# facebookresearch/mbrl-lib

Measured on AMD Instinct MI355X. Metric: candidate-steps/sec (pop×particles×horizon / plan) per CEM iter; plans/sec, higher is better.
Workload: dtype f32

## Files before the change

### __graft_entry__.py

```python
import os
import subprocess
import sys

ROOT = os.path.dirname(os.path.abspath(__file__))
PKG = os.path.join(ROOT, "mbrl-lib_amd")
CSRC = os.path.join(PKG, "csrc")
LIB = os.path.join(PKG, "hipets", "libhipets.so")
BUILDINFO = os.path.join(PKG, "hipets", "libhipets.buildinfo.json")
OBJDIR = os.path.join(PKG, "build")
HIPCC = os.environ.get("HIPCC", "/opt/rocm/bin/hipcc")
HOST_UNITS = ["train.hip", "plan.hip", "rollout.hip", "model.hip", "comm.hip", "engine.hip"]
UNITS = ["rollout_r3.hip", "rollout_r4_gen.hip", "rollout_r4_gens.hip", "rollout_r3_gen.hip", "rollout_r3_gens.hip", "rollout_r2.hip", "rollout_r2_gen.hip",
         "rollout_r2_gens.hip", "rollout_r1_gen.hip", "rollout_r1_gens.hip", "rollout_r1.hip", "rollout_r4.hip", "rollout_r2_fast.hip", "rollout_r3_fast.hip",
         "rollout_r1_fast.hip", "planet.hip"] + HOST_UNITS + ["rollout_r4_fast.hip"]
FLAGS = ["--offload-arch=gfx950", "-O3", "-std=c++17", "-ffp-contract=off", "-fPIC", "-Wno-pass-failed"]


def _sources():
    return sorted(os.path.join(CSRC, f) for f in os.listdir(CSRC)) + [os.path.join(ROOT, "include", "hipets.h")]


def source_digest(extra_flags=()):
    import hashlib

# ... 209 lines not shown
            if "argument unused during compilation" not in line:
                print(line, file=sys.stderr)
        if proc.returncode != 0:
            raise subprocess.CalledProcessError(proc.returncode, cmd)
        stem = os.path.basename(o)[:-2]
        for f in os.listdir(objdir):
            if (f.startswith(stem + "-") or f.startswith(stem + ".")) and f != stem + ".o":
                path = os.path.join(objdir, f)
                if f.endswith("gfx950.s"):
                    resources.update(parse_kernel_resources(path))
                    n, found = scan_isa_hazards(path)
                    isa["asm_mfmas"] += n
                    isa["hazards"] += found
                    isa["units_scanned"].append(u)
                os.remove(path)

    with ThreadPoolExecutor(max_workers=min(len(UNITS), os.cpu_count() or 1)) as ex:
        list(ex.map(lambda uo: compile_unit(*uo), zip(UNITS, objs)))
    link_extra = [f for f in extra_flags if f.startswith("-fsanitize") or f in ("-fno-gpu-sanitize", "-shared-libsan")]
    cmd = [HIPCC, "--offload-arch=gfx950", "-shared", "-fPIC"] + link_extra + objs + ["-o", out]
    print("[build]", " ".join(cmd), flush=True)
    subprocess.run(cmd, check=True)
    with open(os.path.splitext(out)[0] + ".buildinfo.json", "w") as f:
        json.dump({"source_digest": digest, "flags": FLAGS + list(extra_flags), "units": UNITS, "kernels": resources, "isa": isa}, f)
    for h in isa["hazards"][:20]:
        print("[build] ISA HAZARD:", h, file=sys.stderr)
    if isa["hazards"] and not os.environ.get("HIPETS_ALLOW_ISA_HAZARDS") and "-O1" not in extra_flags:
        raise RuntimeError(f"{len(isa['hazards'])} ISA hazard finding(s) in {out}: see {os.path.splitext(out)[0]}.buildinfo.json")
    return digest


DEBUG_LIB = os.path.join(PKG, "hipets", "libhipets_debug.so")
ASAN_LIB = os.path.join(PKG, "hipets", "libhipets_asan.so")
DEBUG_OBJDIR = os.path.join(PKG, "build_debug")
DEBUG_FLAGS = ["-O1", "-gline-tables-only", "-DHIPETS_DEBUG_BOUNDS=1"]
ASAN_FLAGS = ["-fsanitize=address", "-fno-gpu-sanitize", "-shared-libsan", "-Wno-option-ignored"]


def asan_runtime() -> str:
    out = subprocess.run([HIPCC, "--print-file-name=libclang_rt.asan-x86_64.so"], capture_output=True, text=True).stdout.strip()
    if not os.path.isabs(out) or not os.path.exists(out):
        import glob

        found = sorted(glob.glob("/opt/rocm/lib/llvm/lib/clang/*/lib/linux/libclang_rt.asan-x86_64.so"))
        out = found[-1] if found else out
    return out


def build_debug(force: bool = False) -> str:
    import json

    digest = source_digest(DEBUG_FLAGS)
    rebuilt = built_digest(DEBUG_LIB) != digest or force
    build_library(out=DEBUG_LIB, extra_flags=DEBUG_FLAGS, objdir=DEBUG_OBJDIR, force=force)
    asan_digest = source_digest(DEBUG_FLAGS + ASAN_FLAGS)
    if rebuilt or built_digest(ASAN_LIB) != asan_digest:
        from concurrent.futures import ThreadPoolExecutor

        def compile_asan(u):
            obj = os.path.join(DEBUG_OBJDIR, u.replace(".hip", "_asan.o"))
            cmd = [HIPCC] + FLAGS + DEBUG_FLAGS + ASAN_FLAGS + ["-c", os.path.join(CSRC, u), "-o", obj]
            print("[build]", " ".join(cmd), flush=True)
            subprocess.run(cmd, check=True)
            return obj

        with ThreadPoolExecutor(max_workers=min(len(HOST_UNITS), os.cpu_count() or 1)) as ex:
            objs = list(ex.map(compile_asan, HOST_UNITS))
        others = [os.path.join(DEBUG_OBJDIR, u.replace(".hip", ".o")) for u in UNITS if u not in HOST_UNITS]
        cmd = [HIPCC, "--offload-arch=gfx950", "-shared", "-fPIC", "-fsanitize=address", "-fno-gpu-sanitize", "-shared-libsan"] + objs + others + ["-o", ASAN_LIB]
        print("[build]", " ".join(cmd), flush=True)
        subprocess.run(cmd, check=True)
        with open(os.path.splitext(ASAN_LIB)[0] + ".buildinfo.json", "w") as f:
            json.dump({"source_digest": asan_digest, "flags": FLAGS + DEBUG_FLAGS + ASAN_FLAGS, "units": UNITS}, f)
    return DEBUG_LIB


def build(force: bool = False, debug: bool = True) -> None:
    build_library(force=force)
    if debug and os.environ.get("HIPETS_BUILD_DEBUG", "1") != "0":
        build_debug(force)
    build_c_client(force)
    build_fake_rccl(force)
    build_residency_harness(force)
    for p in (PKG, ROOT):
        if p not in sys.path:
            sys.path.insert(0, p)
    import hipets
    from hipets import _lib

    _lib.load()
    from oracle import pets_oracle


C_CLIENT_SRC = os.path.join(ROOT, "tests", "c_abi", "plan_from_c.c")
C_CLIENT = os.path.join(ROOT, "tests", "c_abi", "plan_from_c")


def build_c_client(force: bool = False) -> None:
    if not force and os.path.exists(C_CLIENT) and os.path.getmtime(C_CLIENT) >= max(os.path.getmtime(C_CLIENT_SRC), os.path.getmtime(LIB)):
        return
    cmd = ["gcc", "-std=c99", "-Wall", "-Wextra", "-Werror", "-O1", C_CLIENT_SRC, "-I" + os.path.join(ROOT, "include"),
           "-I/opt/rocm/include", "-D__HIP_PLATFORM_AMD__", "-L" + os.path.dirname(LIB), "-lhipets", "-L/opt/rocm/lib",
           "-lamdhip64", "-lm", "-Wl,-rpath,$ORIGIN/../../mbrl-lib_amd/hipets", "-Wl,-rpath,/opt/rocm/lib", "-o", C_CLIENT]
    print("[build]", " ".join(cmd), flush=True)
    subprocess.run(cmd, check=True)


FAKE_RCCL_SRC = os.path.join(ROOT, "tests", "fake_rccl", "fake_rccl.cpp")
FAKE_RCCL = os.path.join(ROOT, "tests", "fake_rccl", "libfake_rccl.so")


def build_fake_rccl(force: bool = False) -> str:
    if force or not os.path.exists(FAKE_RCCL) or os.path.getmtime(FAKE_RCCL) < os.path.getmtime(FAKE_RCCL_SRC):
        cmd = ["g++", "-std=c++17", "-shared", "-fPIC", "-O1", "-Wall", "-Wextra", FAKE_RCCL_SRC, "-I/opt/rocm/include",
               "-D__HIP_PLATFORM_AMD__", "-L/opt/rocm/lib", "-lamdhip64", "-lrt", "-lpthread", "-Wl,-rpath,/opt/rocm/lib", "-o", FAKE_RCCL]
        print("[build]", " ".join(cmd), flush=True)
        subprocess.run(cmd, check=True)
    return FAKE_RCCL


RESIDENCY_HARNESS_SRC = os.path.join(ROOT, "tests", "residency", "rule_harness.cpp")
RESIDENCY_HARNESS = os.path.join(ROOT, "tests", "residency", "rule_harness")


def build_residency_harness(force: bool = False) -> str:
    srcs = [RESIDENCY_HARNESS_SRC, os.path.join(CSRC, "residency_rule.hpp")]
    if force or not os.path.exists(RESIDENCY_HARNESS) or os.path.getmtime(RESIDENCY_HARNESS) < max(os.path.getmtime(f) for f in srcs):
        cmd = ["g++", "-std=c++17", "-O1", "-g", "-Wall", "-Wextra", "-Werror", "-fsanitize=address,undefined", "-fno-sanitize-recover=all",
               RESIDENCY_HARNESS_SRC, "-o", RESIDENCY_HARNESS]
        print("[build]", " ".join(cmd), flush=True)
        subprocess.run(cmd, check=True)
    return RESIDENCY_HARNESS


def smoke() -> None:
    for p in (PKG, ROOT):
        if p not in sys.path:
            sys.path.insert(0, p)
    import numpy as np
    import torch

    import hipets
    from oracle import pets_oracle as po

    assert torch.cuda.is_available(), "smoke() needs cuda:0"
    dev = "cuda:0"
    obs, act, pop, P, H = 17, 6, 40, 5, 6
    om = po.make_synthetic_model(obs, act, ensemble_size=5, hid=200, seed=0)
    spec = hipets.ModelSpec(weights=om.weights, biases=om.biases, obs_dim=obs, act_dim=act, min_logvar=om.min_logvar,
                            max_logvar=om.max_logvar, norm_mean=om.norm_mean, norm_std=om.norm_std)
    eng = hipets.get_engine(dev)
    eng.set_model(spec)
    g = torch.Generator().manual_seed(0)
    actions = torch.rand(pop, H, act, generator=g) * 2 - 1
    s0 = np.zeros(obs, np.float32)
    perms = torch.stack([torch.randperm(pop * P, generator=g) for _ in range(H)])
    eps = torch.randn(H, pop * P, obs, generator=g)
    out = eng.rollout(actions.to(dev), s0, P, mode="exact", perms=perms.to(dev), eps=eps.to(dev))
    ref = po.rollout(om, actions, s0, P, perms=perms, eps=eps)
    err = (out.cpu() - ref).abs().max().item()
    assert err < 1e-4, f"rollout parity failed: {err}"
    opt = hipets.CEMOptimizer(3, 0.1, 100, [[-1.0] * act] * H, [[1.0] * act] * H, 0.1, dev, return_mean_elites=True, seed=0)
    agent_fn = hipets.make_eval_fn(spec, P, engine=eng)
    from hipets.planning import _BoundObjective

    plan = opt.optimize(_BoundObjective(agent_fn, s0), x0=torch.zeros(H, act))
    torch.cuda.synchronize()
    assert torch.isfinite(plan).all()
    lib = hipets.LIB_PATH
    flags = {os.path.abspath(DEBUG_LIB): DEBUG_FLAGS, os.path.abspath(ASAN_LIB): DEBUG_FLAGS + ASAN_FLAGS}.get(os.path.abspath(lib), ())
    stale = "" if built_digest(lib) == source_digest(flags) else "  ** STALE BINARY: library digest != source digest **"
    print(f"[smoke] rollout max|err| vs oracle = {err:.2e}; fused CEM plan ok; lib = {lib} "
          f"(source digest {built_digest(lib)}){stale}")
    assert not stale, f"{lib} was not built from this source tree"


if __name__ == "__main__":
    build(force="--force" in sys.argv, debug="--no-debug" not in sys.argv)
    if "--smoke" in sys.argv:
        smoke()
```

### mbrl-lib_amd/csrc/cem.hpp

```cpp
#pragma once
#include <type_traits>

#include "common.hpp"

namespace hipets {

struct CemDev {
    int n_env;
    int pop, H, A, D;
    int K;
    float alpha, one_minus_alpha;
    int return_mean, clipped, unbiased;
    const float* totals = nullptr;
    int P = 0;
    const int* elite_in = nullptr;
};

__device__ __forceinline__ float philox_trunc_normal(uint32_t idx_lo, uint32_t idx_hi, uint64_t seed, uint64_t stream) {
    for (uint32_t attempt = 0; attempt < 64; ++attempt) {
        const Philox4 r = philox4x32_10(idx_lo, idx_hi, attempt, (uint32_t)stream, (uint32_t)seed,
                                        (uint32_t)(seed >> 32) ^ (uint32_t)(stream >> 32) ^ 0x5EED5EEDu);
        float n0, n1, n2, n3;
        box_muller(r.x, r.y, n0, n1);
        if (fabsf(n0) <= 2.0f) return n0;
        if (fabsf(n1) <= 2.0f) return n1;
        box_muller(r.z, r.w, n2, n3);
        if (fabsf(n2) <= 2.0f) return n2;
        if (fabsf(n3) <= 2.0f) return n3;
    }
    return 0.0f;
}

__device__ __forceinline__ float philox_normal(uint32_t idx_lo, uint32_t idx_hi, uint64_t seed, uint64_t stream) {
    const Philox4 r = philox4x32_10(idx_lo, idx_hi, 0u, (uint32_t)stream, (uint32_t)seed,
                                    (uint32_t)(seed >> 32) ^ (uint32_t)(stream >> 32) ^ 0x5EED5EEDu);
    float n0, n1;
    box_muller(r.x, r.y, n0, n1);
    return n0;
}

__global__ void cem_sample_kernel(const CemDev p, const float* __restrict__ mu, const float* __restrict__ disp,
                                  const float* __restrict__ lower, const float* __restrict__ upper,
                                  const float* __restrict__ z_in, unsigned long long seed, unsigned long long stream,
                                  float* __restrict__ population) {
    const long long i = (long long)blockIdx.x * blockDim.x + threadIdx.x;
    if (i >= (long long)p.n_env * p.pop * p.D) return;
    const int d = (int)(i % p.D);
    const int env = (int)(i / ((long long)p.pop * p.D));
    const float m = mu[env * p.D + d], v = disp[env * p.D + d], lb = lower[d], ub = upper[d];
    float x;
    if (p.clipped) {
        const float z = z_in ? z_in[i] : philox_normal((uint32_t)i, (uint32_t)(i >> 32), seed, stream);
        x = m + v * z;
        x = x > lb ? x : lb;
        x = x < ub ? x : ub;
    } else {
        const float lbd = (m - lb) / 2.0f, ubd = (ub - m) / 2.0f;
        const float mv = fminf(lbd * lbd, ubd * ubd);
        const float cv = fminf(mv, v);
        const float z = z_in ? z_in[i] : philox_trunc_normal((uint32_t)i, (uint32_t)(i >> 32), seed, stream);
        x = z * sqrtf(cv) + m;
    }
    population[i] = x;
}

#ifndef HIPETS_REFIT_SKIP
#define HIPETS_REFIT_SKIP 0
#endif
constexpr int kRefitThreads = 1024;
constexpr int kMaxPop = 8192;
constexpr int kRefitScratchBytes = 12288;
constexpr int kSelectMaxK = 1024;
constexpr int kRankSortMax = 640;

__global__ __launch_bounds__(kRefitThreads) void cem_refit_kernel(const CemDev p, float* values, const float* population, float* mu,
                                                                 float* disp, float* best_value, float* best_solution,
                                                                 int* elite_idx_out) {
    extern __shared__ __attribute__((aligned(16))) char smem[];
    {
        const int env = blockIdx.y;
        values += (size_t)env * p.pop;
        if (p.totals && !(HIPETS_REFIT_SKIP & 1)) {
            const float* tot = p.totals + (size_t)env * p.pop * p.P;
            for (int i = threadIdx.x; i < p.pop; i += kRefitThreads) {
                float s = 0.f;
                for (int q0 = 0; q0 < p.P; q0 += 8) {
                    float tv[8];
#pragma unroll
                    for (int u = 0; u < 8; ++u) tv[u] = tot[(size_t)i * p.P + min(q0 + u, p.P - 1)];
#pragma unroll
                    for (int u = 0; u < 8; ++u)
                        if (q0 + u < p.P) s += tv[u];
                }
                values[i] = s / (float)p.P;
            }
        }
        population += (size_t)env * p.pop * p.D;
        mu += (size_t)env * p.D;
        disp += (size_t)env * p.D;
        best_value += env;
        best_solution += (size_t)env * p.D;
        if (elite_idx_out) elite_idx_out += (size_t)env * p.K;
    }
    const int* const elite_in = p.elite_in ? p.elite_in + (size_t)blockIdx.y * p.K : nullptr;
    int n2 = 1;
    while (n2 < p.pop) n2 <<= 1;
    float* key = reinterpret_cast<float*>(smem);
    int* idx = reinterpret_cast<int*>(smem + (size_t)n2 * 4);
    const int tid = threadIdx.x;
    for (int i = tid; i < n2; i += kRefitThreads) {
        float v = -INFINITY;
        if (i < p.pop) {
            v = values[i];
            if (v != v) { v = -1e-10f; values[i] = v; }
        }
        key[i] = v;
        idx[i] = i < p.pop ? i : 0x7FFFFFFF;
    }
    __syncthreads();
    if (elite_in) {
        auto in_range = [&](const int e) { return e < 0 ? 0 : (e >= p.pop ? p.pop - 1 : e); };
        const float top_key = key[in_range(elite_in[0])];
        __syncthreads();
        for (int k = tid; k < p.K; k += kRefitThreads) idx[k] = in_range(elite_in[k]);
        if (tid == 0) key[0] = top_key;
        __syncthreads();
    } else if (HIPETS_REFIT_SKIP & 2) {
    } else if (p.pop <= kRankSortMax) {
        for (int i = tid; i < p.pop; i += kRefitThreads) {
            const float ki = key[i];
            int rank = 0;
#pragma unroll 8
            for (int j = 0; j < i; ++j) rank += key[j] >= ki;
#pragma unroll 8
            for (int j = i + 1; j < p.pop; ++j) rank += key[j] > ki;
            idx[i] = rank;
        }
        __syncthreads();
        int* pos = reinterpret_cast<int*>(smem + (size_t)n2 * 8);
        for (int i = tid; i < p.pop; i += kRefitThreads) pos[idx[i]] = i;
        __syncthreads();
        float top_key = key[pos[0]];
        __syncthreads();
        for (int i = tid; i < p.pop; i += kRefitThreads) idx[i] = pos[i];
        if (tid == 0) key[0] = top_key;
        __syncthreads();
    } else if (p.K <= kSelectMaxK) {
        int* hist = reinterpret_cast<int*>(smem + (size_t)n2 * 8);
        int* ctl = hist + 256;
        int* elist = ctl + 8;
        float* ekey = reinterpret_cast<float*>(elist + kSelectMaxK);
        auto okey = [](float v) {
            const unsigned u = __float_as_uint(v + 0.0f);
            return (u & 0x80000000u) ? ~u : (u | 0x80000000u);
        };
        if (tid == 0) { ctl[0] = 0; ctl[1] = 0; ctl[2] = p.K; ctl[3] = 0; }
        for (int pass = 3; pass >= 0; --pass) {
            for (int b = tid; b < 256; b += kRefitThreads) hist[b] = 0;
            __syncthreads();
            const unsigned prefix = (unsigned)ctl[0], mask = (unsigned)ctl[1];
            for (int i = tid; i < p.pop; i += kRefitThreads) {
                const unsigned u = okey(key[i]);
                if ((u & mask) == prefix) atomicAdd(&hist[(u >> (8 * pass)) & 255u], 1);
            }
            __syncthreads();
            if (tid < 64) {
                const int h0 = hist[4 * tid], h1 = hist[4 * tid + 1], h2 = hist[4 * tid + 2], h3 = hist[4 * tid + 3];
                const int mine = h0 + h1 + h2 + h3;
                int above = mine;
#pragma unroll
                for (int d = 1; d < 64; d <<= 1) {
                    const int o = __shfl_down(above, d, 64);
                    if (tid + d < 64) above += o;
                }
                const int need = ctl[2];
                const int higher = above - mine;
                if (higher < need && need <= above) {
                    int n = need - higher, b = 4 * tid + 3;
                    if (n > h3) { n -= h3; b = 4 * tid + 2;
                        if (n > h2) { n -= h2; b = 4 * tid + 1;
                            if (n > h1) { n -= h1; b = 4 * tid; } } }
                    ctl[0] = (int)(prefix | ((unsigned)b << (8 * pass)));
                    ctl[1] = (int)(mask | (255u << (8 * pass)));
                    ctl[2] = n;
                }
            }
            __syncthreads();
        }
        const unsigned T = (unsigned)ctl[0];
        const int need_eq = ctl[2];
        const bool all_eq = hist[T & 255u] == need_eq;
        for (int i = tid; i < p.pop; i += kRefitThreads) {
            const unsigned u = okey(key[i]);
            bool elite = u > T || (u == T && all_eq);
            if (u == T && !all_eq) {
                int before = 0;
                for (int j = 0; j < i; ++j) before += okey(key[j]) == T;
                elite = before < need_eq;
            }
            if (elite) {
                const int slot = atomicAdd(&ctl[3], 1);
                elist[slot] = i;
                ekey[slot] = key[i];
            }
        }
        __syncthreads();
        int my_pos = -1, my_id = 0;
        float my_key = 0.f;
        if (tid < p.K) {
            my_id = elist[tid];
            my_key = ekey[tid];
            int rank = 0;
            for (int f = 0; f < p.K; ++f) {
                const float kf = ekey[f];
                rank += (kf > my_key) || (kf == my_key && elist[f] < my_id);
            }
            my_pos = rank;
        }
        __syncthreads();
        if (my_pos >= 0) idx[my_pos] = my_id;
        if (my_pos == 0) key[0] = my_key;
        __syncthreads();
    } else
    for (int k = 2; k <= n2; k <<= 1) {
        for (int j = k >> 1; j > 0; j >>= 1) {
            for (int i = tid; i < n2; i += kRefitThreads) {
                const int ixj = i ^ j;
                if (ixj > i) {
                    const float ka = key[i], kb = key[ixj];
                    const int ia = idx[i], ib = idx[ixj];
                    const bool a_first = (ka > kb) || (ka == kb && ia < ib);
                    const bool up = (i & k) == 0;
                    if (up ? !a_first : a_first) {
                        key[i] = kb; key[ixj] = ka;
                        idx[i] = ib; idx[ixj] = ia;
                    }
                }
            }
            __syncthreads();
        }
    }
    if (elite_idx_out && blockIdx.x == 0)
        for (int k = tid; k < p.K; k += kRefitThreads) elite_idx_out[k] = idx[k];

    const float top = key[0];
    const bool improved = blockIdx.x == 0 && top > best_value[0];
    const int top_i = idx[0];
    __syncthreads();

    double* red = reinterpret_cast<double*>(smem + (size_t)n2 * 8);
    const int nb = (int)gridDim.x, bx = (int)blockIdx.x;
    const int Dslice = (((p.D + nb - 1) / nb + 63) / 64) * 64;
    const int d_lo = bx * Dslice, d_hi = min(p.D, d_lo + Dslice);
    int parts = kRefitThreads / Dslice;
    parts = parts < 1 ? 1 : (parts > 8 ? 8 : parts);
    const int G = kRefitThreads / parts;
    const int part = tid / G, dloc = tid % G;
    const int nu = (p.K + parts - 1) / parts;
    auto sweep = [&](const int base, auto nu_tag, auto hold_tag) __attribute__((always_inline)) {
        constexpr int NU = decltype(nu_tag)::value;
        constexpr bool HOLD = decltype(hold_tag)::value;
        const int d = base + dloc;
        const bool live = d < d_hi && part < parts;
        float mu_old = 0.f, disp_old = 0.f;
        float xv[NU];
        double s = 0.0;
        if (live) {
            if (part == 0) { mu_old = mu[d]; disp_old = disp[d]; }
            for (int k0 = part; k0 < (HOLD ? part + 1 : p.K); k0 += parts * NU) {
#pragma unroll
                for (int u = 0; u < NU; ++u) xv[u] = population[(size_t)idx[min(k0 + u * parts, p.K - 1)] * p.D + d];
#pragma unroll
                for (int u = 0; u < NU; ++u)
                    if (k0 + u * parts < p.K) s += (double)xv[u];
            }
        }
        red[tid] = s;
        __syncthreads();
        double mean = 0.0;
        if (live) {
            for (int q = 0; q < parts; ++q) mean += red[q * G + dloc];
            mean /= (double)p.K;
        }
        __syncthreads();
        double ss = 0.0;
        if (live) {
            for (int k0 = part; k0 < (HOLD ? part + 1 : p.K); k0 += parts * NU) {
                if constexpr (!HOLD) {
#pragma unroll
                    for (int u = 0; u < NU; ++u) xv[u] = population[(size_t)idx[min(k0 + u * parts, p.K - 1)] * p.D + d];
                }
#pragma unroll
                for (int u = 0; u < NU; ++u)
                    if (k0 + u * parts < p.K) {
                        const double dv = (double)xv[u] - mean;
                        ss += dv * dv;
                    }
            }
        }
        red[tid] = ss;
        __syncthreads();
        if (live && part == 0) {
            double var = 0.0;
            for (int q = 0; q < parts; ++q) var += red[q * G + dloc];
            var /= (double)(p.unbiased ? (p.K - 1) : p.K);
            const float new_mu = (float)mean;
            const float new_disp = p.clipped ? (float)sqrt(var) : (float)var;
            mu[d] = p.alpha * mu_old + p.one_minus_alpha * new_mu;
            disp[d] = p.alpha * disp_old + p.one_minus_alpha * new_disp;
        }
        __syncthreads();
    };
    constexpr int kBestHold = 4;
    float best_row[kBestHold];
    const bool best_held = p.D <= kBestHold * kRefitThreads;
    if (improved && best_held) {
#pragma unroll
        for (int u = 0; u < kBestHold; ++u) best_row[u] = population[(size_t)top_i * p.D + min(tid + u * kRefitThreads, p.D - 1)];
    }
    for (int base = d_lo; base < ((HIPETS_REFIT_SKIP & 4) ? d_lo : d_hi); base += G) {
        using T = std::true_type;
        using F = std::false_type;
        if (nu <= 2) sweep(base, std::integral_constant<int, 2>{}, T{});
        else if (nu <= 4) sweep(base, std::integral_constant<int, 4>{}, T{});
        else if (nu <= 8) sweep(base, std::integral_constant<int, 8>{}, T{});
        else if (nu <= 16) sweep(base, std::integral_constant<int, 16>{}, T{});
        else sweep(base, std::integral_constant<int, 16>{}, F{});
    }
    if (improved) {
        if (best_held) {
#pragma unroll
            for (int u = 0; u < kBestHold; ++u)
                if (tid + u * kRefitThreads < p.D) best_solution[tid + u * kRefitThreads] = best_row[u];
        } else {
            for (int d = tid; d < p.D; d += kRefitThreads) best_solution[d] = population[(size_t)top_i * p.D + d];
        }
        if (tid == 0) best_value[0] = top;
    }
}

inline int refit_blocks(const int D) { return D <= 128 ? 1 : (D + 127) / 128 > 8 ? 8 : (D + 127) / 128; }

__global__ void cem_init_kernel(const CemDev p, const float* x0, const float* lower, const float* upper, float* mu,
                                float* disp, float* best_value) {
    const int i = blockIdx.x * blockDim.x + threadIdx.x;
    if (i < p.n_env * p.D) {
        const int d = i % p.D;
        mu[i] = x0[i];
        const float w = upper[d] - lower[d];
        disp[i] = p.clipped ? 1.0f : (w * w) / 16.0f;
    }
    if (i < p.n_env) best_value[i] = -INFINITY;
}

}
```

### mbrl-lib_amd/csrc/plan.hip

```cpp
#include <algorithm>
#include <cmath>
#include <vector>

#include "engine.hpp"
#include "lds_optin.hpp"
#include "optim.hpp"

using namespace hipets;

namespace {

int launch_mppi_sample(int n_env, int pop, int H, int A, float beta, const float* mean, const float* past_action, const float* lower, const float* upper,
                       const float* z, uint64_t seed, uint64_t stream_id, float* population, hipStream_t st) {
    const long long npop = (long long)n_env * pop;
    const long long D = (long long)H * A;
    if (D <= kMppiSampleMaxD) {
        const int G = mppi_sample_group(npop, (int)D);
        hipLaunchKernelGGL(mppi_sample_staged_kernel, dim3((unsigned)((npop + G - 1) / G)), dim3(kMppiSampleThreads), (size_t)G * D * 4, st, n_env, pop, H, A, G, beta,
                           mean, past_action, lower, upper, z, (unsigned long long)seed, (unsigned long long)stream_id, population);
    } else {
        const long long n = npop * A;
        hipLaunchKernelGGL(mppi_sample_kernel, dim3((unsigned)((n + 255) / 256)), dim3(256), 0, st, n_env, pop, H, A, beta, mean, past_action, lower, upper, z,
                           (unsigned long long)seed, (unsigned long long)stream_id, population);
    }
// ... 93 lines not shown
    if (le->ok()) le->note(rollout_impl(e, population + (size_t)lo * nd, nullptr, hi - lo, H, P, ro, shard_out, stream));
    if (world > 1) {
        hipStream_t st = reinterpret_cast<hipStream_t>(stream);
        if (comm_all_gather(e, (size_t)width, st)) return 1;
        if (le->ok()) le->note(comm_unpad_shards(e, rows, width, st));
    }
    return 0;
}

struct PlanObjective {
    enum Kind { ENSEMBLE, SHARDED, PLANET } kind = ENSEMBLE;
    const float* s0 = nullptr;
    const float* latent0 = nullptr;
    const float* belief0 = nullptr;

    bool is_planet() const { return kind == PLANET; }
    bool is_sharded() const { return kind == SHARDED; }
    uint64_t rollout_seed(const hipets_engine* e, uint64_t seed) const {
        return seed + (is_sharded() ? (uint64_t)e->comm_rank : 0ull) * 0x9E3779B97F4A7C15ull;
    }
    size_t shard_width(const hipets_engine* e, int max_rows) const { return (size_t)((max_rows + e->comm_world - 1) / e->comm_world); }
    int reserve_shards(hipets_engine* e, int max_rows) const {
        if (!is_sharded()) return 0;
        const size_t width = shard_width(e, max_rows);
        return e->shard_values.ensure(width * 4) || e->gathered.ensure((size_t)e->comm_world * width * 4);
    }
    int clear_padding(hipets_engine* e, int max_rows, hipStream_t st) const {
        if (is_sharded()) HCHECK(hipMemsetAsync(e->shard_values.p, 0, shard_width(e, max_rows) * 4, st));
        return 0;
    }
    void refit_from_totals(hipets_engine* e, CemDev* c, int P) const {
        if (is_sharded()) return;
        c->totals = e->totals.as<float>();
        c->P = P;
    }
    int evaluate(hipets_engine* e, const float* population, int rows, int H, int P, const hipets_rollout_opts* ro, float* returns,
                 void* stream, LocalErr& le) const {
        if (is_sharded()) return sharded_evaluate(e, population, rows, H, P, ro, stream, &le);
        if (!le.ok()) return 0;
        if (!is_planet()) {
            le.note(rollout_impl(e, population, nullptr, rows, H, P, ro, returns, stream));
            return 0;
        }
        hipets_planet_opts po{};
        po.seed = ro->seed;
        po.stream_id = ro->stream_id;
        po.n_env = ro->n_env;
        le.note(planet_rollout_impl(e, population, latent0, belief0, rows, H, P, &po, returns, reinterpret_cast<hipStream_t>(stream)));
        return 0;
    }
};
PlanObjective ensemble_objective(const float* s0, PlanObjective::Kind kind = PlanObjective::ENSEMBLE) {
    PlanObjective o;
    o.kind = kind;
    o.s0 = s0;
    return o;
}
PlanObjective planet_objective(const float* latent0, const float* belief0) {
    PlanObjective o;
    o.kind = PlanObjective::PLANET;
    o.latent0 = latent0;
    o.belief0 = belief0;
    return o;
}

int check_plan(const hipets_engine* e, const PlanObjective& obj, bool args, int A, int n_env, int P) {
    const bool planet = obj.is_planet();
    if (planet && !(e && e->has_planet)) return fail("engine has no PlaNet model (call hipets_planet_set_model)");
    if (!planet && !(e && e->has_model)) return fail("engine has no model (call hipets_set_model)");
    if (!args || (planet ? !(obj.latent0 && obj.belief0) : !obj.s0)) return fail("null argument");
    if (planet && A != e->pd.action) return fail("act_dim %d != model action_size %d", A, e->pd.action);
    if (!planet && A != e->md.act_dim) return fail("act_dim %d != model act_dim %d", A, e->md.act_dim);
    if (n_env < 1 || n_env > 4096) return fail("n_env %d outside [1, 4096]", n_env);
    if (planet && P < 1) return fail("bad pop/horizon/particles");
    return 0;
}

int launch_cem_refit(const CemDev& c, float* values, const float* population, float* mu, float* disp, float* best_value, float* best_solution,
                     int* elite_idx, hipStream_t st) {
    int n2 = 1;
    while (n2 < c.pop) n2 <<= 1;
    hipLaunchKernelGGL(cem_refit_kernel, dim3(refit_blocks(c.D), c.n_env), dim3(kRefitThreads), (size_t)n2 * 8 + kRefitScratchBytes, st, c, values,
                       population, mu, disp, best_value, best_solution, elite_idx);
    HCHECK(hipGetLastError());
    return 0;
}

struct PlanLoop {
    int n_env, H, P, iters;
    uint64_t first_stream, stream_stride, rollout_stream;
    const float* population;
    float* returns;
};
template <class Prologue, class Rows, class Sample, class Refit>
int run_plan(hipets_engine* e, const PlanObjective& obj, const PlanLoop& pl, uint64_t seed, void* stream, Prologue prologue, Rows rows, Sample sample,
             Refit refit) {
    hipets_rollout_opts ro{};
    ro.mode = e->plan_mode;
    ro.seed = obj.rollout_seed(e, seed);
    ro.n_env = pl.n_env;
    const bool carry_on = obj.is_sharded();
    LocalErr le;
    le.note(prologue(ro.seed));
    for (int i = 0; i < pl.iters && (carry_on || le.ok()); ++i) {
        const uint64_t sid = (pl.first_stream + (uint64_t)i) * pl.stream_stride;
        if (le.ok()) le.note(sample(i, sid));
        ro.stream_id = sid + pl.rollout_stream;
        if (obj.evaluate(e, pl.population, rows(i), pl.H, pl.P, &ro, pl.returns, stream, le)) return 1;
        if (le.ok()) le.note(refit(i));
    }
    return le.report();
}

int plan_cem_impl(hipets_engine* e, const hipets_cem_params* p, int32_t n_env, const float* x0, const float* lower, const float* upper,
                  const PlanObjective& obj, int32_t P, uint64_t seed, uint64_t plan_id, float* out, void* stream) {
    if (check_cem(p) || check_plan(e, obj, x0 && lower && upper && out, p->act_dim, n_env, P)) return 1;
    if (obj.is_sharded() && check_shards(e, p->population_size, P)) return 1;
    hipStream_t st = reinterpret_cast<hipStream_t>(stream);
    HCHECK(hipSetDevice(e->device));
    ENTER_STREAM(e, st);
    const CemDev c = make_cem(p, n_env);
    const size_t nd = (size_t)n_env * c.D, npop = (size_t)n_env * c.pop;
    if (e->mu.ensure(nd * 4) || e->disp.ensure(nd * 4) || e->best_solution.ensure(nd * 4) || e->best_value.ensure((size_t)n_env * 4 + 16) ||
        e->population.ensure(npop * c.D * 4) || e->values.ensure(npop * 4) || obj.reserve_shards(e, c.pop))
        return 1;
    const int iters = p->num_iterations;
    const PlanLoop pl{n_env, c.H, P, iters, plan_id * (uint64_t)iters, 1, 0, e->population.as<float>(), nullptr};
    auto prologue = [&](uint64_t rollout_seed) -> int {
        if (obj.clear_padding(e, c.pop, st)) return 1;
        hipLaunchKernelGGL(cem_init_kernel, dim3((unsigned)((nd + 255) / 256)), dim3(256), 0, st, c, x0, lower, upper, e->mu.as<float>(),
                           e->disp.as<float>(), e->best_value.as<float>());
        HCHECK(hipGetLastError());
        HCHECK(hipMemsetAsync(e->best_solution.p, 0, nd * 4, st));
        return obj.is_planet() ? 0 : plan_prologue(e, obj.s0, n_env, c.H, iters, rollout_seed, pl.first_stream, st);
    };
    auto sample = [&](int, uint64_t sid) -> int {
        const long long n = (long long)npop * c.D;
        hipLaunchKernelGGL(cem_sample_kernel, dim3((unsigned)((n + 255) / 256)), dim3(256), 0, st, c, e->mu.as<float>(), e->disp.as<float>(),
                           lower, upper, (const float*)nullptr, (unsigned long long)seed, (unsigned long long)sid, e->population.as<float>());
        HCHECK(hipGetLastError());
        return 0;
    };
    auto refit = [&](int i) -> int {
        int* eidx = (e->has_trace && e->trace.elite_idx) ? e->trace.elite_idx + (size_t)i * n_env * c.K : nullptr;
        CemDev cr = c;
        obj.refit_from_totals(e, &cr, P);
        if (launch_cem_refit(cr, e->values.as<float>(), e->population.as<float>(), e->mu.as<float>(), e->disp.as<float>(), e->best_value.as<float>(),
                             e->best_solution.as<float>(), eidx, st))
            return 1;
        return trace_iter(e, i, (int)npop, (size_t)c.D, e->population.as<float>(), e->values.as<float>(), e->mu.as<float>(), e->disp.as<float>(), st, n_env);
    };
    if (run_plan(e, obj, pl, seed, stream, prologue, [&](int) { return (int)npop; }, sample, refit)) return 1;
    HCHECK(hipMemcpyAsync(out, p->return_mean_elites ? e->mu.p : e->best_solution.p, nd * 4, hipMemcpyDeviceToDevice, st));
    return 0;
}

int plan_mppi_impl(hipets_engine* e, int32_t pop, int32_t H, int32_t A, int32_t num_iterations, double gamma, double beta, int32_t n_env,
                   float* mean, const float* lower, const float* upper, const PlanObjective& obj, int32_t P, uint64_t seed, uint64_t plan_id,
                   void* stream) {
    if (check_plan(e, obj, mean && lower && upper, A, n_env, P)) return 1;
    if (pop < 1 || pop > 12000) return fail("population_size %d outside [1, 12000]", pop);
    if (H < 1 || num_iterations < 0) return fail("bad horizon/num_iterations");
    if (obj.is_sharded() && check_shards(e, pop, P)) return 1;
    hipStream_t st = reinterpret_cast<hipStream_t>(stream);
    HCHECK(hipSetDevice(e->device));
    ENTER_STREAM(e, st);
    const size_t nd = (size_t)H * A, npop = (size_t)n_env * pop;
    if (e->mu.ensure(n_env * nd * 4) || e->past_action.ensure((size_t)n_env * A * 4) || e->population.ensure(npop * nd * 4) ||
        e->values.ensure(npop * 4) || obj.reserve_shards(e, pop))
        return 1;
    const PlanLoop pl{n_env, H, P, num_iterations, plan_id * (uint64_t)num_iterations, 1, 0, e->population.as<float>(), e->values.as<float>()};
    auto prologue = [&](uint64_t rollout_seed) -> int {
        if (obj.clear_padding(e, pop, st)) return 1;
        HCHECK(hipMemcpyAsync(e->mu.p, mean, n_env * nd * 4, hipMemcpyDeviceToDevice, st));
        hipLaunchKernelGGL(mppi_shift_kernel, dim3((unsigned)((n_env * nd + 255) / 256)), dim3(256), 0, st, n_env, H, A, e->mu.as<float>(), mean,
                           e->past_action.as<float>());
        HCHECK(hipGetLastError());
        return obj.is_planet() ? 0 : plan_prologue(e, obj.s0, n_env, H, num_iterations, rollout_seed, pl.first_stream, st);
    };
    auto sample = [&](int, uint64_t sid) -> int {
        return launch_mppi_sample(n_env, pop, H, A, (float)beta, mean, e->past_action.as<float>(), lower, upper, nullptr, seed, sid,
                                  e->population.as<float>(), st);
    };
    auto update = [&](int k) -> int {
        if (launch_mppi_update(e, n_env, pop, (int)nd, (float)gamma, e->values.as<float>(), e->population.as<float>(), mean, st)) return 1;
        return trace_iter(e, k, (int)npop, nd, e->population.as<float>(), e->values.as<float>(), mean, nullptr, st, n_env);
    };
    return run_plan(e, obj, pl, seed, stream, prologue, [&](int) { return (int)npop; }, sample, update);
}

int plan_icem_impl(hipets_engine* e, const hipets_icem_params* p, int32_t n_env, const float* x0, const float* lower, const float* upper,
                   float* elite, int32_t has_elite, const int32_t* keep_idx, const PlanObjective& obj, int32_t P, uint64_t seed, uint64_t plan_id,
                   float* out, void* stream) {
    if (check_plan(e, obj, p && x0 && lower && upper && elite && out, p ? p->act_dim : 0, n_env, P)) return 1;
    if (p->horizon < 2 || p->horizon > kMaxHorizon) return fail("iCEM horizon %d outside [2, %d]", p->horizon, kMaxHorizon);
    const int K = p->elite_num, keep = p->keep_elite_size, iters = p->num_iterations, H = p->horizon, A = p->act_dim;
    if (K < 1 || keep < 0 || keep > K) return fail("elite_num %d / keep_elite_size %d invalid", K, keep);
    if (p->population_size < 1 || iters < 0 || !(p->population_decay_factor > 0.0)) return fail("bad iCEM parameters");
    std::vector<int> sizes(iters), rows_of(iters);
    int max_rows = 1;
    for (int i = 0, he = has_elite; i < iters; ++i, he = 1) {
        int n = (int)std::ceil(std::fmax((double)p->population_size * std::pow(p->population_decay_factor, -(double)i), 2.0 * K));
        const int m = p->population_size_module;
        if (m > 0 && n % m) n += m - n % m;
        sizes[i] = n;
        if (n + keep > kMaxPop) return fail("iCEM iteration %d evaluates %d candidates (max %d)", i, n + keep, kMaxPop);
        rows_of[i] = n + (he ? ((i == iters - 1 && i != 0) ? 1 : keep) : 0);
        if (K > rows_of[i]) return fail("elite_num %d invalid", K);
        max_rows = std::max(max_rows, n + keep);
        if (obj.is_sharded() && check_shards(e, rows_of[i], P)) return 1;
    }
    hipStream_t st = reinterpret_cast<hipStream_t>(stream);
    HCHECK(hipSetDevice(e->device));
    ENTER_STREAM(e, st);
    const size_t nd = (size_t)H * A, ne = (size_t)n_env;
    if (e->mu.ensure(ne * nd * 4) || e->disp.ensure(ne * nd * 4) || e->best_solution.ensure(ne * nd * 4) || e->best_value.ensure(ne * 4 + 16) ||
        e->population.ensure(ne * max_rows * nd * 4) || e->values.ensure(ne * max_rows * 4) ||
        e->kept.ensure(ne * std::max(keep, 1) * nd * 4) || e->elite_idx.ensure(ne * K * 4) || e->keep_idx.ensure(ne * std::max(keep, 1) * 4) ||
        (!obj.is_planet() && e->s0.ensure(ne * e->md.obs_dim * 4)) || obj.reserve_shards(e, max_rows))
        return 1;
    hipets_cem_params cp{};
    cp.population_size = std::max(K, 1);
    cp.horizon = H;
    cp.act_dim = A;
    cp.num_iterations = iters;
    cp.elite_num = K;
    cp.alpha = p->alpha;
    cp.return_mean_elites = p->return_mean_elites;
    cp.clipped_normal = 0;
    cp.unbiased_var = 0;
    float* popbuf = e->population.as<float>();
    const PlanLoop pl{n_env, H, P, iters, plan_id * (uint64_t)iters, 4, 3, popbuf, nullptr};
    auto prologue = [&](uint64_t) -> int {
        if (obj.clear_padding(e, max_rows, st)) return 1;
        hipLaunchKernelGGL(cem_init_kernel, dim3((unsigned)((ne * nd + 255) / 256)), dim3(256), 0, st, make_cem(&cp, n_env), x0, lower, upper,
                           e->mu.as<float>(), e->disp.as<float>(), e->best_value.as<float>());
// ... 237 lines not shown
```

Measured before the change: 289.8 million.

## Fuse CEM refit with next-iteration sampling and final output into one boundary kernel

Adds a boundary kernel that computes particle means, elite selection, mean/dispersion update, best-solution tracking and sampling of the next population in one launch. This replaces the separate sample kernel, the refit kernel and the final device copy. A start kernel merges init, the best_solution memset and the first sampling. best_value becomes double-buffered by iteration parity so that several blocks can read and write it without racing. The goal is fewer kernel launches per CEM iteration, at the cost of having every block redo the sort and particle-mean work and of having fewer threads sample the population.

```diff
diff --git a/__graft_entry__.py b/__graft_entry__.py
--- a/__graft_entry__.py
+++ b/__graft_entry__.py
@@ -315,6 +315,7 @@
     build_c_client(force)
     build_fake_rccl(force)
     build_residency_harness(force)
+    build_boundary_harness(force)
     for p in (PKG, ROOT):
         if p not in sys.path:
             sys.path.insert(0, p)
@@ -364,6 +365,20 @@
         print("[build]", " ".join(cmd), flush=True)
         subprocess.run(cmd, check=True)
     return RESIDENCY_HARNESS
+
+
+BOUNDARY_HARNESS_SRC = os.path.join(ROOT, "tests", "cem_boundary", "rule_harness.cpp")
+BOUNDARY_HARNESS = os.path.join(ROOT, "tests", "cem_boundary", "rule_harness")
+
+
+def build_boundary_harness(force: bool = False) -> str:
+    srcs = [BOUNDARY_HARNESS_SRC, os.path.join(CSRC, "cem_boundary_rule.hpp")]
+    if force or not os.path.exists(BOUNDARY_HARNESS) or os.path.getmtime(BOUNDARY_HARNESS) < max(os.path.getmtime(f) for f in srcs):
+        cmd = ["g++", "-std=c++17", "-O1", "-g", "-Wall", "-Wextra", "-Werror", "-fsanitize=address,undefined", "-fno-sanitize-recover=all",
+               BOUNDARY_HARNESS_SRC, "-o", BOUNDARY_HARNESS]
+        print("[build]", " ".join(cmd), flush=True)
+        subprocess.run(cmd, check=True)
+    return BOUNDARY_HARNESS
 
 
 def smoke() -> None:
diff --git a/mbrl-lib_amd/csrc/cem.hpp b/mbrl-lib_amd/csrc/cem.hpp
--- a/mbrl-lib_amd/csrc/cem.hpp
+++ b/mbrl-lib_amd/csrc/cem.hpp
@@ -1,6 +1,7 @@
 #pragma once
 #include <type_traits>
 
+#include "cem_boundary_rule.hpp"
 #include "common.hpp"
 
 namespace hipets {
@@ -39,6 +40,21 @@
     return n0;
 }
 
+__device__ __forceinline__ float cem_candidate(const int clipped, const float m, const float v, const float lb, const float ub, const long long i,
+                                               const float* __restrict__ z_in, const unsigned long long seed, const unsigned long long stream) {
+    if (clipped) {
+        const float z = z_in ? z_in[i] : philox_normal((uint32_t)i, (uint32_t)(i >> 32), seed, stream);
+        float x = m + v * z;
+        x = x > lb ? x : lb;
+        return x < ub ? x : ub;
+    }
+    const float lbd = (m - lb) / 2.0f, ubd = (ub - m) / 2.0f;
+    const float mv = fminf(lbd * lbd, ubd * ubd);
+    const float cv = fminf(mv, v);
+    const float z = z_in ? z_in[i] : philox_trunc_normal((uint32_t)i, (uint32_t)(i >> 32), seed, stream);
+    return z * sqrtf(cv) + m;
+}
+
 __global__ void cem_sample_kernel(const CemDev p, const float* __restrict__ mu, const float* __restrict__ disp,
                                   const float* __restrict__ lower, const float* __restrict__ upper,
                                   const float* __restrict__ z_in, unsigned long long seed, unsigned long long stream,
@@ -47,53 +63,53 @@
     if (i >= (long long)p.n_env * p.pop * p.D) return;
     const int d = (int)(i % p.D);
     const int env = (int)(i / ((long long)p.pop * p.D));
-    const float m = mu[env * p.D + d], v = disp[env * p.D + d], lb = lower[d], ub = upper[d];
-    float x;
-    if (p.clipped) {
-        const float z = z_in ? z_in[i] : philox_normal((uint32_t)i, (uint32_t)(i >> 32), seed, stream);
-        x = m + v * z;
-        x = x > lb ? x : lb;
-        x = x < ub ? x : ub;
-    } else {
-        const float lbd = (m - lb) / 2.0f, ubd = (ub - m) / 2.0f;
-        const float mv = fminf(lbd * lbd, ubd * ubd);
-        const float cv = fminf(mv, v);
-        const float z = z_in ? z_in[i] : philox_trunc_normal((uint32_t)i, (uint32_t)(i >> 32), seed, stream);
-        x = z * sqrtf(cv) + m;
-    }
-    population[i] = x;
+    population[i] = cem_candidate(p.clipped, mu[env * p.D + d], disp[env * p.D + d], lower[d], upper[d], i, z_in, seed, stream);
 }
 
 #ifndef HIPETS_REFIT_SKIP
 #define HIPETS_REFIT_SKIP 0
 #endif
-constexpr int kRefitThreads = 1024;
 constexpr int kMaxPop = 8192;
 constexpr int kRefitScratchBytes = 12288;
 constexpr int kSelectMaxK = 1024;
 constexpr int kRankSortMax = 640;
 
-__global__ __launch_bounds__(kRefitThreads) void cem_refit_kernel(const CemDev p, float* values, const float* population, float* mu,
-                                                                 float* disp, float* best_value, float* best_solution,
-                                                                 int* elite_idx_out) {
+
+struct CemBoundary {
+    int width = 0;
+    int parity = 0;
+    int last = 0;
+    const float* lower = nullptr;
+    const float* upper = nullptr;
+    unsigned long long seed = 0, stream = 0;
+    float* next = nullptr;
+    float* out = nullptr;
+};
+
+template <bool BOUNDARY>
+__device__ __forceinline__ void cem_refit_body(const CemDev& p, const CemBoundary& b, float* values, const float* population, float* mu,
+                                               float* disp, float* best_value, float* best_solution, int* elite_idx_out) {
     extern __shared__ __attribute__((aligned(16))) char smem[];
+    const float* tot = nullptr;
+    auto particle_mean = [&](const int i) {
+        float s = 0.f;
+        for (int q0 = 0; q0 < p.P; q0 += 8) {
+            float tv[8];
+#pragma unroll
+            for (int u = 0; u < 8; ++u) tv[u] = tot[(size_t)i * p.P + min(q0 + u, p.P - 1)];
+#pragma unroll
+            for (int u = 0; u < 8; ++u)
+                if (q0 + u < p.P) s += tv[u];
+        }
+        return s / (float)p.P;
+    };
     {
         const int env = blockIdx.y;
         values += (size_t)env * p.pop;
         if (p.totals && !(HIPETS_REFIT_SKIP & 1)) {
-            const float* tot = p.totals + (size_t)env * p.pop * p.P;
-            for (int i = threadIdx.x; i < p.pop; i += kRefitThreads) {
-                float s = 0.f;
-                for (int q0 = 0; q0 < p.P; q0 += 8) {
-                    float tv[8];
-#pragma unroll
-                    for (int u = 0; u < 8; ++u) tv[u] = tot[(size_t)i * p.P + min(q0 + u, p.P - 1)];
-#pragma unroll
-                    for (int u = 0; u < 8; ++u)
-                        if (q0 + u < p.P) s += tv[u];
-                }
-                values[i] = s / (float)p.P;
-            }
+            tot = p.totals + (size_t)env * p.pop * p.P;
+            if constexpr (!BOUNDARY)
+                for (int i = threadIdx.x; i < p.pop; i += kRefitThreads) values[i] = particle_mean(i);
         }
         population += (size_t)env * p.pop * p.D;
         mu += (size_t)env * p.D;
@@ -111,8 +127,14 @@
     for (int i = tid; i < n2; i += kRefitThreads) {
         float v = -INFINITY;
         if (i < p.pop) {
-            v = values[i];
-            if (v != v) { v = -1e-10f; values[i] = v; }
+            if constexpr (BOUNDARY) {
+                v = tot ? particle_mean(i) : values[i];
+                if (v != v) v = -1e-10f;
+                if (blockIdx.x == 0) values[i] = v;
+            } else {
+                v = values[i];
+                if (v != v) { v = -1e-10f; values[i] = v; }
+            }
         }
         key[i] = v;
         idx[i] = i < p.pop ? i : 0x7FFFFFFF;
@@ -244,16 +266,16 @@
         for (int k = tid; k < p.K; k += kRefitThreads) elite_idx_out[k] = idx[k];
 
     const float top = key[0];
-    const bool improved = blockIdx.x == 0 && top > best_value[0];
+    const float best_old = best_value[BOUNDARY ? b.parity * p.n_env : 0];
+    const bool improved = (BOUNDARY || blockIdx.x == 0) && top > best_old;
     const int top_i = idx[0];
     __syncthreads();
 
     double* red = reinterpret_cast<double*>(smem + (size_t)n2 * 8);
     const int nb = (int)gridDim.x, bx = (int)blockIdx.x;
-    const int Dslice = (((p.D + nb - 1) / nb + 63) / 64) * 64;
-    const int d_lo = bx * Dslice, d_hi = min(p.D, d_lo + Dslice);
-    int parts = kRefitThreads / Dslice;
-    parts = parts < 1 ? 1 : (parts > 8 ? 8 : parts);
+    const int Dslice = BOUNDARY ? b.width : refit_slice(p.D, nb);
+    const int d_lo = min(p.D, bx * Dslice), d_hi = min(p.D, d_lo + Dslice);
+    const int parts = BOUNDARY ? refit_parts(p.D) : (kRefitThreads / Dslice < 1 ? 1 : (kRefitThreads / Dslice > 8 ? 8 : kRefitThreads / Dslice));
     const int G = kRefitThreads / parts;
     const int part = tid / G, dloc = tid % G;
     const int nu = (p.K + parts - 1) / parts;
@@ -308,13 +330,22 @@
             const float new_disp = p.clipped ? (float)sqrt(var) : (float)var;
             mu[d] = p.alpha * mu_old + p.one_minus_alpha * new_mu;
             disp[d] = p.alpha * disp_old + p.one_minus_alpha * new_disp;
+            if constexpr (BOUNDARY)
+                if (b.last && p.return_mean) b.out[(size_t)blockIdx.y * p.D + d] = mu[d];
         }
         __syncthreads();
     };
     constexpr int kBestHold = 4;
     float best_row[kBestHold];
     const bool best_held = p.D <= kBestHold * kRefitThreads;
-    if (improved && best_held) {
+    if constexpr (BOUNDARY) {
+        for (int d = d_lo + tid; d < d_hi; d += kRefitThreads) {
+            const float x = improved ? population[(size_t)top_i * p.D + d] : best_solution[d];
+            if (improved) best_solution[d] = x;
+            if (b.last && !p.return_mean) b.out[(size_t)blockIdx.y * p.D + d] = x;
+        }
+        if (bx == 0 && tid == 0) best_value[(b.parity ^ 1) * p.n_env] = improved ? top : best_old;
+    } else if (improved && best_held) {
 #pragma unroll
         for (int u = 0; u < kBestHold; ++u) best_row[u] = population[(size_t)top_i * p.D + min(tid + u * kRefitThreads, p.D - 1)];
     }
@@ -327,6 +358,18 @@
         else if (nu <= 16) sweep(base, std::integral_constant<int, 16>{}, T{});
         else sweep(base, std::integral_constant<int, 16>{}, F{});
     }
+    if constexpr (BOUNDARY) {
+        if (b.last) return;
+        const int w = d_hi - d_lo;
+        float* const next = b.next + (size_t)blockIdx.y * p.pop * p.D;
+        for (int e = tid; e < p.pop * w; e += kRefitThreads) {
+            const int d = d_lo + e % w;
+            const size_t at = (size_t)(e / w) * p.D + d;
+            next[at] = cem_candidate(p.clipped, mu[d], disp[d], b.lower[d], b.upper[d], (long long)((size_t)blockIdx.y * p.pop * p.D + at), nullptr,
+                                     b.seed, b.stream);
+        }
+        return;
+    }
     if (improved) {
         if (best_held) {
 #pragma unroll
@@ -339,7 +382,16 @@
     }
 }
 
-inline int refit_blocks(const int D) { return D <= 128 ? 1 : (D + 127) / 128 > 8 ? 8 : (D + 127) / 128; }
+__global__ __launch_bounds__(kRefitThreads) void cem_refit_kernel(const CemDev p, float* values, const float* population, float* mu,
+                                                                 float* disp, float* best_value, float* best_solution,
+                                                                 int* elite_idx_out) {
+    cem_refit_body<false>(p, CemBoundary{}, values, population, mu, disp, best_value, best_solution, elite_idx_out);
+}
+
+__global__ __launch_bounds__(kRefitThreads) void cem_boundary_kernel(const CemDev p, const CemBoundary b, float* values, float* mu, float* disp,
+                                                                    float* best_value, float* best_solution) {
+    cem_refit_body<true>(p, b, values, b.next, mu, disp, best_value, best_solution, nullptr);
+}
 
 __global__ void cem_init_kernel(const CemDev p, const float* x0, const float* lower, const float* upper, float* mu,
                                 float* disp, float* best_value) {
@@ -353,4 +405,22 @@
     if (i < p.n_env) best_value[i] = -INFINITY;
 }
 
-}
+__global__ void cem_start_kernel(const CemDev p, const float* x0, const float* lower, const float* upper, unsigned long long seed,
+                                 unsigned long long stream, float* mu, float* disp, float* best_value, float* best_solution, float* population) {
+    const long long i = (long long)blockIdx.x * blockDim.x + threadIdx.x;
+    if (i < 2 * p.n_env) best_value[i] = -INFINITY;
+    if (i >= (long long)p.n_env * p.pop * p.D) return;
+    const int d = (int)(i % p.D);
+    const int at = (int)(i / ((long long)p.pop * p.D)) * p.D + d;
+    const float w = upper[d] - lower[d];
+    const float m = x0[at], v = p.clipped ? 1.0f : (w * w) / 16.0f;
+    if (i < (long long)p.n_env * p.D) {
+        mu[i] = x0[i];
+        const float wi = upper[i % p.D] - lower[i % p.D];
+        disp[i] = p.clipped ? 1.0f : (wi * wi) / 16.0f;
+        best_solution[i] = 0.f;
+    }
+    population[i] = cem_candidate(p.clipped, m, v, lower[d], upper[d], i, nullptr, seed, stream);
+}
+
+}
diff --git a/mbrl-lib_amd/csrc/cem_boundary_rule.hpp b/mbrl-lib_amd/csrc/cem_boundary_rule.hpp
--- /dev/null
+++ b/mbrl-lib_amd/csrc/cem_boundary_rule.hpp
@@ -0,0 +1,49 @@
+#pragma once
+
+#if defined(__HIPCC__)
+#define HIPETS_RULE_HD __host__ __device__
+#else
+#define HIPETS_RULE_HD
+#endif
+
+namespace hipets {
+
+constexpr int kRefitThreads = 1024;
+
+HIPETS_RULE_HD inline int refit_blocks(const int D) { return D <= 128 ? 1 : (D + 127) / 128 > 8 ? 8 : (D + 127) / 128; }
+
+HIPETS_RULE_HD inline int refit_slice(const int D, const int nb) { return (((D + nb - 1) / nb + 63) / 64) * 64; }
+
+HIPETS_RULE_HD inline int refit_parts(const int D) {
+    const int parts = kRefitThreads / refit_slice(D, refit_blocks(D));
+    return parts < 1 ? 1 : (parts > 8 ? 8 : parts);
+}
+
+struct BoundaryPlan {
+    bool fused = false;
+    int width = 0;
+    int blocks = 0;
+};
+
+constexpr int kBoundaryDraws = 2048;
+constexpr int kBoundaryBlocks = 256;
+
+inline BoundaryPlan cem_boundary_plan(const bool traced, const bool sharded, const int iters, const int n_env, const int pop, const int D) {
+    BoundaryPlan b;
+    if (traced || sharded || iters < 1 || n_env < 1 || pop < 1 || D < 1) return b;
+    b.fused = true;
+    const int plain = refit_blocks(D), widest = (D + plain - 1) / plain;
+    int width = kBoundaryDraws / pop;
+    width = width < 1 ? 1 : (width > widest ? widest : width);
+    int blocks = (D + width - 1) / width;
+    const int cap = kBoundaryBlocks / n_env > plain ? kBoundaryBlocks / n_env : plain;
+    if (blocks > cap) {
+        width = (D + cap - 1) / cap;
+        blocks = (D + width - 1) / width;
+    }
+    b.width = width;
+    b.blocks = blocks;
+    return b;
+}
+
+}
diff --git a/mbrl-lib_amd/csrc/plan.hip b/mbrl-lib_amd/csrc/plan.hip
--- a/mbrl-lib_amd/csrc/plan.hip
+++ b/mbrl-lib_amd/csrc/plan.hip
@@ -199,6 +199,27 @@
     while (n2 < c.pop) n2 <<= 1;
     hipLaunchKernelGGL(cem_refit_kernel, dim3(refit_blocks(c.D), c.n_env), dim3(kRefitThreads), (size_t)n2 * 8 + kRefitScratchBytes, st, c, values,
                        population, mu, disp, best_value, best_solution, elite_idx);
+    HCHECK(hipGetLastError());
+    return 0;
+}
+
+int launch_cem_boundary(const CemDev& c, const BoundaryPlan& bp, int i, int iters, const float* lower, const float* upper, uint64_t seed, uint64_t next_sid,
+                        float* values, float* population, float* mu, float* disp, float* best_value, float* best_solution, float* out, hipStream_t st) {
+    if (!c.totals) return fail("CEM boundary launch without particle totals");
+    int n2 = 1;
+    while (n2 < c.pop) n2 <<= 1;
+    CemBoundary b;
+    b.width = bp.width;
+    b.parity = i & 1;
+    b.last = i == iters - 1;
+    b.lower = lower;
+    b.upper = upper;
+    b.seed = (unsigned long long)seed;
+    b.stream = (unsigned long long)next_sid;
+    b.next = population;
+    b.out = out;
+    hipLaunchKernelGGL(cem_boundary_kernel, dim3(bp.blocks, c.n_env), dim3(kRefitThreads), (size_t)n2 * 8 + kRefitScratchBytes, st, c, b, values, mu, disp,
+                       best_value, best_solution);
     HCHECK(hipGetLastError());
     return 0;
 }
@@ -238,13 +259,22 @@
     ENTER_STREAM(e, st);
     const CemDev c = make_cem(p, n_env);
     const size_t nd = (size_t)n_env * c.D, npop = (size_t)n_env * c.pop;
-    if (e->mu.ensure(nd * 4) || e->disp.ensure(nd * 4) || e->best_solution.ensure(nd * 4) || e->best_value.ensure((size_t)n_env * 4 + 16) ||
+    if (e->mu.ensure(nd * 4) || e->disp.ensure(nd * 4) || e->best_solution.ensure(nd * 4) || e->best_value.ensure((size_t)n_env * 8 + 16) ||
         e->population.ensure(npop * c.D * 4) || e->values.ensure(npop * 4) || obj.reserve_shards(e, c.pop))
         return 1;
     const int iters = p->num_iterations;
     const PlanLoop pl{n_env, c.H, P, iters, plan_id * (uint64_t)iters, 1, 0, e->population.as<float>(), nullptr};
+    const BoundaryPlan bp = cem_boundary_plan(e->has_trace, obj.is_sharded(), iters, n_env, c.pop, c.D);
     auto prologue = [&](uint64_t rollout_seed) -> int {
         if (obj.clear_padding(e, c.pop, st)) return 1;
+        if (bp.fused) {
+            const long long n = std::max((long long)npop * c.D, 2ll * n_env);
+            hipLaunchKernelGGL(cem_start_kernel, dim3((unsigned)((n + 255) / 256)), dim3(256), 0, st, c, x0, lower, upper, (unsigned long long)seed,
+                               (unsigned long long)pl.first_stream, e->mu.as<float>(), e->disp.as<float>(), e->best_value.as<float>(),
+                               e->best_solution.as<float>(), e->population.as<float>());
+            HCHECK(hipGetLastError());
+            return obj.is_planet() ? 0 : plan_prologue(e, obj.s0, n_env, c.H, iters, rollout_seed, pl.first_stream, st);
+        }
         hipLaunchKernelGGL(cem_init_kernel, dim3((unsigned)((nd + 255) / 256)), dim3(256), 0, st, c, x0, lower, upper, e->mu.as<float>(),
                            e->disp.as<float>(), e->best_value.as<float>());
         HCHECK(hipGetLastError());
@@ -252,6 +282,7 @@
         return obj.is_planet() ? 0 : plan_prologue(e, obj.s0, n_env, c.H, iters, rollout_seed, pl.first_stream, st);
     };
     auto sample = [&](int, uint64_t sid) -> int {
+        if (bp.fused) return 0;
         const long long n = (long long)npop * c.D;
         hipLaunchKernelGGL(cem_sample_kernel, dim3((unsigned)((n + 255) / 256)), dim3(256), 0, st, c, e->mu.as<float>(), e->disp.as<float>(),
                            lower, upper, (const float*)nullptr, (unsigned long long)seed, (unsigned long long)sid, e->population.as<float>());
@@ -262,13 +293,18 @@
         int* eidx = (e->has_trace && e->trace.elite_idx) ? e->trace.elite_idx + (size_t)i * n_env * c.K : nullptr;
         CemDev cr = c;
         obj.refit_from_totals(e, &cr, P);
+        if (bp.fused)
+            return launch_cem_boundary(cr, bp, i, iters, lower, upper, seed, pl.first_stream + (uint64_t)i + 1, e->values.as<float>(),
+                                       e->population.as<float>(), e->mu.as<float>(), e->disp.as<float>(), e->best_value.as<float>(),
+                                       e->best_solution.as<float>(), out, st);
         if (launch_cem_refit(cr, e->values.as<float>(), e->population.as<float>(), e->mu.as<float>(), e->disp.as<float>(), e->best_value.as<float>(),
                              e->best_solution.as<float>(), eidx, st))
             return 1;
         return trace_iter(e, i, (int)npop, (size_t)c.D, e->population.as<float>(), e->values.as<float>(), e->mu.as<float>(), e->disp.as<float>(), st, n_env);
     };
     if (run_plan(e, obj, pl, seed, stream, prologue, [&](int) { return (int)npop; }, sample, refit)) return 1;
-    HCHECK(hipMemcpyAsync(out, p->return_mean_elites ? e->mu.p : e->best_solution.p, nd * 4, hipMemcpyDeviceToDevice, st));
+    if (!bp.fused)
+        HCHECK(hipMemcpyAsync(out, p->return_mean_elites ? e->mu.p : e->best_solution.p, nd * 4, hipMemcpyDeviceToDevice, st));
     return 0;
 }
 
diff --git a/profiles/cem_boundary_summary.py b/profiles/cem_boundary_summary.py
--- /dev/null
+++ b/profiles/cem_boundary_summary.py
@@ -0,0 +1,63 @@
+import csv
+import json
+import os
+import statistics
+import sys
+
+ROOT = os.path.dirname(os.path.dirname(os.path.abspath(__file__)))
+
+
+def kernel_table(path, plans):
+    rows = {}
+    for r in csv.DictReader(open(path)):
+        name = r["Name"].split("(")[0].replace("void ", "").split("<")[0]
+        if name.startswith(("hipets::", "__amd_rocclr")):
+            rows[name] = {"launches_per_plan": round(int(r["Calls"]) / plans, 2), "avg_us": round(float(r["AverageNs"]) / 1e3, 2),
+                          "us_per_plan": round(float(r["TotalDurationNs"]) / 1e3 / plans, 1)}
+    return rows
+
+
+def bench_lines(path):
+    line = [ln for ln in open(path) if ln.startswith('{"metric"')][-1]
+    d = json.loads(line)
+    ex = d.get("extras", d)
+    other = ex["other_configs"]
+    cfg1 = next(v for k, v in other.items() if "cfg1" in k)
+    mode = next(k for k in cfg1 if k != "optimizer")
+    return {"headline ms_per_step": d["ms_per_step"], "cfg1 ms_per_plan": cfg1[mode]["ms_per_plan"], "planet ms_per_plan": ex["planet"]["ms_per_plan"],
+            "pets_cartpole ms_per_plan": ex["stock_defaults"]["pets_cartpole"][mode]["ms_per_plan"]}
+
+
+def verdict(parent, new):
+    spread = max(max(parent) - min(parent), max(new) - min(new))
+    diff = statistics.median(parent) - statistics.median(new)
+    gain = max(new) < min(parent) and diff >= 3 * spread
+    return {"parent": parent, "new": new, "median_parent": statistics.median(parent), "median_new": statistics.median(new), "median_difference": diff,
+            "median_difference_percent": 100 * diff / statistics.median(parent), "larger_spread": spread, "every_new_run_beats_every_parent_run": max(new) < min(parent),
+            "result": "gain" if gain else "no gain by the rule (difference < 3 x spread, or the runs overlap)"}
+
+
+def main():
+    d, ab = sys.argv[1], sys.argv[2]
+    plans = int(sys.argv[3]) if len(sys.argv) > 3 else 25
+    out = {"what": "CEM boundary launches (csrc/cem.hpp cem_boundary_kernel / cem_start_kernel) against the parent commit, MI355X, one box per job",
+           "kernel_trace": {"command": "rocprofv3 --kernel-trace --memory-copy-trace --stats -- python bench.py --steps 20 --no-cpu-baseline --no-extras",
+                            "plans": plans}}
+    for b in ("parent", "new"):
+        t = kernel_table(os.path.join(d, f"trace_{b}", "bench_kernel_stats.csv"), plans)
+        out["kernel_trace"][b] = {"kernels": t, "non_rollout_us_per_plan": round(sum(v["us_per_plan"] for k, v in t.items() if "rollout_kernel" not in k
+                                                                                    and "pack_" not in k), 1),
+                                  "launches_per_plan": round(sum(v["launches_per_plan"] for k, v in t.items() if "pack_" not in k), 2)}
+    runs = {b: [bench_lines(os.path.join(ab, f"{b}{i}.log")) for i in (1, 2, 3)] for b in ("parent", "new")}
+    out["bench"] = {"command": "python bench.py --gpus 1 --steps 50 --no-cpu-baseline, order parent1 new1 parent2 new2 parent3 new3",
+                    "lines": {k: verdict([r[k] for r in runs["parent"]], [r[k] for r in runs["new"]]) for k in runs["parent"][0]}}
+    path = os.path.join(ROOT, "profiles", "cem_boundary.json")
+    if os.path.exists(path) and "rejected" in json.load(open(path)):
+        out["rejected"] = json.load(open(path))["rejected"]
+    json.dump(out, open(path, "w"), indent=1)
+    print(json.dumps(out["bench"], indent=1))
+    print(json.dumps({b: (out["kernel_trace"][b]["non_rollout_us_per_plan"], out["kernel_trace"][b]["launches_per_plan"]) for b in ("parent", "new")}))
+
+
+if __name__ == "__main__":
+    main()
```

Result: no change. 290.1 million, median of 6 (+0.1%).
